# databio/gtars

Measured on AMD Instinct MI355X. Metric: query intervals/sec tokenized vs 100k-region hg38 universe, higher is better.
Workload: dtype u32; 1 GPU; BASELINE config 2: tokenize hg38-shaped query regions vs 100k-region universe (Bits order, CSR u64 offsets + u32 token ids), inputs resident in HBM; universe_regions=100000, distinct_batches=32, resident_bytes_rotated=714602184

## Files before the change

### gtars_amd/csrc/tokenize_lds.hip

```cpp
#include "common.h"
#include "scan.h"

#include <mutex>

namespace gtars {

#ifndef GTARS_TOK_ABLATE
#define GTARS_TOK_ABLATE 0
#endif

__device__ __forceinline__ i64 overlap_bp_tok(u32 as, u32 ae, u32 bs, u32 be) {
    u32 mn = ae < be ? ae : be;
    u32 mx = as > bs ? as : bs;
    return (i64)mn - (i64)mx;
}

typedef u32 u32x4 __attribute__((ext_vector_type(4)));
typedef u32 u32x2 __attribute__((ext_vector_type(2)));
typedef u64 u64x2 __attribute__((ext_vector_type(2)));
__device__ __forceinline__ u32x4 ld_stream4(const u32 *p) { return __builtin_nontemporal_load(reinterpret_cast<const u32x4 *>(p)); }
__device__ __forceinline__ u32x2 ld_stream2(const u32 *p) { return __builtin_nontemporal_load(reinterpret_cast<const u32x2 *>(p)); }
__device__ __forceinline__ void st_stream2(u64 *p, u64 a, u64 b) {
    u64x2 v = {a, b};
    __builtin_nontemporal_store(v, reinterpret_cast<u64x2 *>(p));
}

#ifndef GTARS_TOK_FILL_U
#define GTARS_TOK_FILL_U 4
#endif
#ifndef GTARS_TOK_PRIO
#define GTARS_TOK_PRIO 0
#endif
#ifndef GTARS_TOK_LB_W1
#define GTARS_TOK_LB_W1 1
#endif
#ifndef GTARS_TOK_KEYS_U16
#define GTARS_TOK_KEYS_U16 1
#endif
#ifndef GTARS_TOK_SEARCH8
#define GTARS_TOK_SEARCH8 1
#endif
#ifndef GTARS_TOK_STAMPS
#define GTARS_TOK_STAMPS 0
#endif
#ifndef GTARS_TOK_UNIT2_EXACT
#define GTARS_TOK_UNIT2_EXACT 1
#endif
#if GTARS_TOK_STAMPS
__device__ unsigned long long g_tok_stamps[2][12];
#define TSTAMP(k)                                         \
    do {                                                  \
        const u64 _t = __builtin_amdgcn_s_memtime();      \
        ts_acc[k] += _t - ts_last;                        \
        ts_last = _t;                                     \
    } while (0)
#else
#define TSTAMP(k) \
    do {          \
    } while (0)
#endif

template <bool FILTER>
__device__ __forceinline__ bool hit_test(u32 s, u32 e, u32 qs, u32 qe, i32 min_bp) {
    bool hit = (s < qe) & (e > qs);
    if (FILTER) hit = hit && overlap_bp_tok(qs, qe, s, e) >= (i64)min_bp;
    return hit;
}

template <bool FILTER>
__device__ __forceinline__ u32 block_mask4(const uint4 &S, const uint4 &E, u32 qs, u32 qe, i32 min_bp) {
    u32 m = 0;
    m |= (hit_test<FILTER>(S.x, E.x, qs, qe, min_bp) ? 1u : 0u);
    m |= (hit_test<FILTER>(S.y, E.y, qs, qe, min_bp) ? 1u : 0u) << 1;
    m |= (hit_test<FILTER>(S.z, E.z, qs, qe, min_bp) ? 1u : 0u) << 2;
    m |= (hit_test<FILTER>(S.w, E.w, qs, qe, min_bp) ? 1u : 0u) << 3;
    return m;
}

constexpr u32 B0_BITS = 22;
constexpr u32 B0_MASK = (1u << B0_BITS) - 1u;
__device__ __forceinline__ u32 run_state(u32 n, u32 m) { return (n & B0_MASK) | (m << B0_BITS) | ((n >> B0_BITS) << (B0_BITS + 4)); }
#ifndef GTARS_TOK_STAGE_RUNS
#define GTARS_TOK_STAGE_RUNS 1
#endif
constexpr u32 RUN_Q_BIT = 4, STAB_W_BIT = 8, STAB_N_BIT = 16;
__device__ __forceinline__ u32 run_state_n(u32 st) { return (st & B0_MASK) | ((st >> (B0_BITS + 4)) << B0_BITS); }

template <bool FILTER, u32 STRIDE, class F>
__device__ __forceinline__ u32 walk_tail(const uint4 *__restrict__ recs, u32 b0, u32 be, u32 qs, u32 qe, i32 min_bp, F &&f) {
    static_assert(ACC_OWN == 2, "a record = two own intervals + two look-ahead intervals");
    u32 n = 0;
    bool mr = true;
    for (u32 b = b0 + 2; mr && b < be; b += 2) {
        const uint4 S = recs[(size_t)b * STRIDE], E = recs[(size_t)b * STRIDE + 1];
        u32 m = block_mask4<FILTER>(S, E, qs, qe, min_bp);
        mr = S.w < qe;
        n += __popc(m);
        while (m) {
            const int k = __ffs((int)m) - 1;
            m &= m - 1;
            f(b, k);
        }
    }
    return n;
}

template <int SUB, bool IN_UNIT = true>
__device__ __forceinline__ void search_blocks(const AccelView &a, const u32 *s_lut, const u32 *s_q, const uint4 *s_ctab,
// ... 541 lines not shown
                }
            }
        } else {
            i = __popc(m);
        }
        if (more && want_ids) {
            const u32 n_tail = walk_tail<FILTER, STRIDE>(recs, b_tail, be, sq, eq, min_bp, [&](u32 b, int k) {
                put(slot(i++), IMPL ? t.aux[IMPL ? j : 0] + (u32)ACC_OWN * (b - b0) + (u32)k : recw[b * 16u + 8u + (u32)k]);
            });
            if (!tail_counted) n_all += n_tail;
        }
        run += n_all;
    }
}

template <int QPT, bool REV>
__device__ __forceinline__ void coop_runs(const TileQ<QPT, true> &t, const u64 (&o4)[QPT], u64 wave_base, u32 *__restrict__ ovals,
                                          u64 cap, int lane) {
    static_assert(QPT == 4, "four runs per source lane");
    u32 S[QPT], N[QPT], K[QPT];
    u32 any_big = 0;
#pragma unroll
    for (int j = 0; j < QPT; ++j) {
        const u32 m = (t.st[j] >> B0_BITS) & 15u, pm = __popc(m), w = (t.more_bits >> (STAB_W_BIT + 2 * j)) & 3u,
                  n_stab = (t.more_bits >> (STAB_N_BIT + 4 * j)) & 15u;
        const bool joined = w == 0 && mask_joins_tail(m);
        const u32 n = run_state_n(t.st[j]) + (joined ? pm : 0u);
        const bool big = ((t.more_bits >> (RUN_Q_BIT + j)) & 1u) && n >= COOP_MIN;
        S[j] = (u32)(o4[j] - wave_base) + (REV || joined ? 0u : pm + n_stab);
        N[j] = big ? n : 0u;
        const u32 id0 = joined ? t.aux[j] + (u32)(__ffs((int)m) - 1) : t.aux[j] + 4u + 4u * w;
        K[j] = REV ? id0 + (n - 1u) + S[j] : id0 - S[j];
        any_big |= N[j];
    }
    unsigned long long todo = __ballot(any_big != 0);
    if (!todo || wave_base >= cap) return;
    u32 *__restrict__ out = ovals + wave_base;
    const u32 room = cap - wave_base > 0xFFFFFFFFull ? 0xFFFFFFFFu : (u32)(cap - wave_base);
    u32 w0 = 0, val = 0;
    bool has = false;
    bool open = false;
    while (todo) {
        const int src = __ffsll((long long)todo) - 1;
        todo &= todo - 1;
        u32 s_[QPT], n_[QPT], k_[QPT];
#pragma unroll
        for (int j = 0; j < QPT; ++j) {
            s_[j] = (u32)__builtin_amdgcn_readlane((int)S[j], src);
            n_[j] = (u32)__builtin_amdgcn_readlane((int)N[j], src);
            k_[j] = (u32)__builtin_amdgcn_readlane((int)K[j], src);
        }
        u32 lo = 0xFFFFFFFFu, hi = 0;
#pragma unroll
        for (int j = 0; j < QPT; ++j)
            if (n_[j]) {
                lo = lo < s_[j] ? lo : s_[j];
                hi = s_[j] + n_[j];
            }
        hi = hi < room ? hi : room;
        for (u32 w = lo & ~63u; w < hi; w += 64) {
            if (w != w0) {
                if (open && has) __builtin_nontemporal_store(val, &out[w0 + (u32)lane]);
                has = false;
                w0 = w;
            }
            open = true;
            const u32 x = w + (u32)lane;
#pragma unroll
            for (int j = 0; j < QPT; ++j) {
                const bool in = x - s_[j] < n_[j];
                val = in ? (REV ? k_[j] - x : k_[j] + x) : val;
                has = has || in;
            }
            has = has && x < room;
        }
    }
    if (open && has) __builtin_nontemporal_store(val, &out[w0 + (u32)lane]);
}

template <int QPT, bool FILTER, bool IMPL, bool REV, int RUNS, bool U64 = false>
__device__ __forceinline__ void write_queries(const AccelView &a, const SearchLds &L, const u32 *__restrict__ qc,
                                              const u32 *__restrict__ qs, const u32 *__restrict__ qe, u64 nq, i32 min_bp,
                                              const TileQ<QPT, IMPL> &t, u64 q0, u64 wave_base, u64 *__restrict__ offsets,
                                              u32 *__restrict__ ovals, u64 cap, bool off_vec_ok, u32 *stage, u32 stage_cap,
                                              int lane) {
    const bool staged = cap && t.wtotal <= stage_cap && wave_base + t.wtotal <= cap;
    u64 o4[QPT];
    emit_queries<QPT, FILTER, IMPL, REV, RUNS, U64>(a, L, qc, qs, qe, min_bp, t, q0, wave_base + t.excl, cap != 0, o4, !staged, [&](u64 pos, u32 id) {
        if (GTARS_TOK_ABLATE & 2) return;
        if (staged)
            stage[(u32)(pos - wave_base)] = id;
        else if (pos < cap)
            ovals[pos] = id;
    });
    if constexpr (IMPL && !FILTER && (RUNS & 4) != 0) {
        if (!staged && cap && a.runs_ok && !(GTARS_TOK_ABLATE & (2 | 128))) coop_runs<QPT, REV>(t, o4, wave_base, ovals, cap, lane);
    }
    if (staged && !(GTARS_TOK_ABLATE & 2)) {
        for (u32 i = (u32)lane; i < t.wtotal; i += 64) __builtin_nontemporal_store(stage[i], &ovals[wave_base + i]);
    }
    if (GTARS_TOK_ABLATE & 4) {
        if (o4[0] == 0xFFFFFFFFFFFFFFFFull) offsets[q0] = o4[QPT - 1];
    } else if (QPT >= 2 && off_vec_ok && q0 + QPT <= nq) {
#pragma unroll
        for (int h = 0; h < QPT / 2; ++h) st_stream2(offsets + q0 + 2 * h, o4[2 * h], o4[2 * h + 1]);
    } else {
#pragma unroll
        for (int j = 0; j < QPT; ++j)
            if (q0 + j < nq) offsets[q0 + j] = o4[j];
    }
}

template <int QPT, bool FILTER, bool IMPL, bool REV, int RUNS, bool U64 = false>
__device__ __forceinline__ bool stage_queries(const AccelView &a, const SearchLds &L, const u32 *__restrict__ qc,
                                              const u32 *__restrict__ qs, const u32 *__restrict__ qe, i32 min_bp,
                                              const TileQ<QPT, IMPL> &t, u64 q0, u64 cap, u32 *stage, u32 stage_cap,
                                              u32 (&orel)[QPT]) {
    if (cap && t.wtotal > stage_cap) return false;
#if !GTARS_TOK_STAGE_RUNS
    if (IMPL && !FILTER && (RUNS & 1) && __ballot((t.more_bits >> RUN_Q_BIT) & 15u)) return false;
#endif
    u64 o4[QPT];
    emit_queries<QPT, FILTER, IMPL, REV, (GTARS_TOK_STAGE_RUNS != 0 ? RUNS : 0), U64>(a, L, qc, qs, qe, min_bp, t, q0, (u64)t.excl, cap != 0, o4, false, [&](u64 pos, u32 id) {
        if (GTARS_TOK_ABLATE & 2) return;
        stage[(u32)pos] = id;
    });
#pragma unroll
    for (int j = 0; j < QPT; ++j) orel[j] = (u32)o4[j];
    return true;
}
template <int QPT>
__device__ __forceinline__ void flush_queries(u64 nq, u32 wtotal, const u32 (&orel)[QPT], u64 q0, u64 wave_base,
                                              u64 *__restrict__ offsets, u32 *__restrict__ ovals, u64 cap, bool off_vec_ok,
                                              const u32 *stage, int lane) {
    if (cap && !(GTARS_TOK_ABLATE & 2)) {
        const u32 n = wave_base >= cap ? 0u : (cap - wave_base < (u64)wtotal ? (u32)(cap - wave_base) : wtotal);
        for (u32 i = (u32)lane; i < n; i += 64) __builtin_nontemporal_store(stage[i], &ovals[wave_base + i]);
    }
    if (GTARS_TOK_ABLATE & 4) {
        if (orel[0] == 0xFFFFFFFFu) offsets[q0] = orel[QPT - 1];
    } else if (QPT >= 2 && off_vec_ok && q0 + QPT <= nq) {
#pragma unroll
        for (int h = 0; h < QPT / 2; ++h) st_stream2(offsets + q0 + 2 * h, wave_base + orel[2 * h], wave_base + orel[2 * h + 1]);
    } else {
#pragma unroll
        for (int j = 0; j < QPT; ++j)
            if (q0 + j < nq) offsets[q0 + j] = wave_base + orel[j];
    }
}

template <bool FILTER>
__device__ __forceinline__ u64 help_count_tile(const AccelView &a, const SearchLds &L, const u32 *qc, const u32 *qs,
                                               const u32 *qe, u64 q_begin, u64 q_end, i32 min_bp) {
    u64 n = 0;
    for (u64 q = q_begin + (threadIdx.x & 63); q < q_end; q += 64) {
        const u32 c = qc[q], s = qs[q], e = qe[q];
        u32 b0, be;
        search_blocks<1>(a, L.lut, L.q, L.ctab, &c, &s, &b0, &be);
        if (b0 < be) {
            const uint4 S = a.rec2[(size_t)b0 * 2], E = a.rec2[(size_t)b0 * 2 + 1];
            n += __popc(block_mask4<FILTER>(S, E, s, e, min_bp));
            if (S.w < e && b0 + 2 < be) n += walk_tail<FILTER, 2>(a.rec2, b0, be, s, e, min_bp, [](u32, int) {});
        }
    }
    return wave_reduce_sum_u64(n);
}

template <int W, class Help>
__device__ __forceinline__ u64 resolve_prefix_helping(u64 *state, u32 tile, u64 agg, int lane, u32 epoch, u32 spin_limit,
                                                      u64 base, Help &&help) {
    const u64 ep = (u64)epoch << EP_SHIFT;
    u64 part = 0;
    i64 pred = (i64)tile - 1;
    u32 spins = 0;
    bool done = pred < 0;
    auto load_window = [&](i64 first) -> u64 {
        const i64 idx = first - lane;
        u64 v = ST_INC;
        if (idx >= 0) {
            v = ld_state(&state[idx]);
            if ((u32)((v >> EP_SHIFT) & EP_MAX) != epoch) v = 0;
        }
        return v;
    };
    while (!done) {
#if GTARS_TOK_STAMPS
        if (lane == 0) atomicAdd(&g_tok_stamps[1][spins ? 9 : 8], 1ull);
#endif
        u64 v[W];
#pragma unroll
        for (int w = 0; w < W; ++w) v[w] = load_window(pred - 64 * w);
#pragma unroll
        for (int w = 0; w < W; ++w) {
            if (done) continue;
            for (;;) {
                const u64 status = v[w] & ST_MASK;
                const unsigned long long b_inc = __ballot(status == ST_INC);
                const unsigned long long b_inv = __ballot(status == 0);
                const int first_inc = b_inc ? __ffsll((long long)b_inc) - 1 : 64;
                const unsigned long long need = first_inc >= 63 ? ~0ull : ((1ull << (first_inc + 1)) - 1ull);
                if (!(b_inv & need)) {
                    part += lane <= first_inc ? (v[w] & VAL_MASK) : 0ull;
                    if (first_inc < 64) done = true;
                    break;
                }
                if (++spins > spin_limit) {
                    const i64 missing = pred - 64 * w - (__ffsll((long long)(b_inv & need)) - 1);
                    const u64 h = help((u32)missing) + (missing == 0 ? base : 0ull);
                    if (lane == 0) st_state(&state[missing], (missing == 0 ? ST_INC : ST_AGG) | ep | h);
                    spins = 0;
                } else {
                    __builtin_amdgcn_s_sleep(1);
                }
                v[w] = load_window(pred - 64 * w);
            }
        }
        pred -= 64 * W;
        if (pred < 0) done = true;
    }
    const u64 excl = wave_reduce_sum_u48(part) + (tile == 0 ? base : 0ull);
    if (lane == 0) st_state(&state[tile], ST_INC | ep | (excl + agg));
    return excl;
}

__device__ __forceinline__ void group_barrier(u32 *ctr, u32 &phase, u32 members, int lane) {
    asm volatile("s_waitcnt lgkmcnt(0)" ::: "memory");
    phase += members;
    if (lane == 0) __hip_atomic_fetch_add(ctr, 1u, __ATOMIC_RELAXED, __HIP_MEMORY_SCOPE_WORKGROUP);
    for (;;) {
        const u32 v = __builtin_amdgcn_readfirstlane(__hip_atomic_load(ctr, __ATOMIC_RELAXED, __HIP_MEMORY_SCOPE_WORKGROUP));
        if ((i32)(v - phase) >= 0) break;
        __builtin_amdgcn_s_sleep(1);
    }
    asm volatile("" ::: "memory");
}

template <int TPB, int QPT, int R, int G, bool FILTER, bool IMPL, bool REV, int RUNS, bool U64 = false>
__global__ void __launch_bounds__(TPB, TPB / 256)
k_tok_lds(AccelView a, const u32 *__restrict__ qc, const u32 *__restrict__ qs, const u32 *__restrict__ qe,
          u64 nq, i32 min_bp, u64 *__restrict__ offsets, u32 *__restrict__ ovals, u64 cap, ScanWs *ws,
          u32 epoch, u32 ticket_base, u32 stage_cap, u32 spin_limit, const u64 *__restrict__ d_base,
          u64 *__restrict__ d_total_out) {
    extern __shared__ __attribute__((aligned(16))) u32 smem[];
    constexpr int NW = TPB / 64, GW = NW / G;
    static_assert(GW * R <= 64, "one lane per wave part in the group's scan");
    __shared__ u32 s_tile[G];
    __shared__ u64 s_prefix[G];
    __shared__ u32 s_scan[G][GW * R];
    __shared__ u32 s_bar[G];
    constexpr u32 ROUND = GW * 64 * QPT;
    constexpr u32 TILE = ROUND * R;

    const u32 num_tiles = (u32)((nq + TILE - 1) / TILE);
    const int lane = threadIdx.x & 63;
    const int wave = __builtin_amdgcn_readfirstlane(threadIdx.x >> 6);
    const int grp = wave / GW, gwave = wave % GW;
    const u32 gtid = threadIdx.x - (u32)grp * GW * 64;
    const u32 first_tiles = gridDim.x * G;
    const bool vec_ok = ((((uintptr_t)qc) | ((uintptr_t)qs) | ((uintptr_t)qe)) & 15u) == 0;
    const bool off_vec_ok = (((uintptr_t)offsets) & 15u) == 0;
    const SearchLds L = search_lds_view(a, smem);
    u32 *stage = smem + tok_lds_bytes(a) / 4 + (size_t)wave * stage_cap;
    const u64 base = d_base ? *d_base : 0ull;

    u32 c[R][QPT], s[R][QPT], e[R][QPT];
    auto load_tile = [&](u32 t) {
#pragma unroll
        for (int r = 0; r < R; ++r)
            load_queries<QPT>(qc, qs, qe, nq, (u64)t * TILE + (u64)r * ROUND + (u64)gtid * QPT, vec_ok, c[r], s[r], e[r]);
    };
    u32 tile = blockIdx.x * G + (u32)grp;
    load_tile(tile);
    if (G > 1 && threadIdx.x < G) s_bar[threadIdx.x] = 0;
    if (!(GTARS_TOK_ABLATE & 32)) fill_search_lds<TPB>(a, smem);
    __syncthreads();

    u32 phase = 0;
    auto bar = [&]() {
        if constexpr (G == 1)
            lds_barrier();
        else
            group_barrier(&s_bar[grp], phase, (u32)GW, lane);
    };
    auto help = [&](u32 t) -> u64 {
        const u64 qb = (u64)t * TILE, qn = qb + TILE < nq ? qb + TILE : nq;
        return help_count_tile<FILTER>(a, L, qc, qs, qe, qb, qn, min_bp);
    };

    struct Prev {
        TileQ<QPT, IMPL> q[R];
        u32 wbase[R], total, tile;
    } cur, prev;
    bool have_prev = false, loaded = true;
    const bool draw = num_tiles > first_tiles;
#if GTARS_TOK_STAMPS
    u64 ts_acc[12] = {0, 0, 0, 0, 0, 0, 0, 0, 0, 0, 0, 0}, ts_last = __builtin_amdgcn_s_memtime();
#endif
    for (;;) {
        const bool has_cur = tile < num_tiles;
        u32 next_tile = num_tiles;
        if (has_cur) {
            u32 ticket = 0;
            if (draw && gtid == 0) ticket = atomicAdd(&ws->ticket, 1u);
            if (!loaded) load_tile(tile);
            loaded = false;
#if GTARS_TOK_STAMPS
            asm volatile("s_waitcnt vmcnt(0)" ::: "memory");
#endif
            TSTAMP(0);
            u32 tsum[R], inc[R];
#if GTARS_TOK_PRIO & 1
            __builtin_amdgcn_s_setprio(1);
#endif
            count_rounds<R, QPT, FILTER, IMPL, REV, RUNS, U64>(a, L, c, s, e, min_bp, cur.q, tsum);
#if GTARS_TOK_PRIO & 1
            __builtin_amdgcn_s_setprio(0);
#endif
            TSTAMP(1);
#pragma unroll
            for (int r = 0; r < R; ++r) {
                inc[r] = wave_inclusive_scan_u32(tsum[r], lane);
                if (lane == 63) s_scan[grp][r * GW + gwave] = inc[r];
            }
            if (draw && gtid == 0) s_tile[grp] = first_tiles + (ticket - ticket_base);
            bar();
            TSTAMP(2);
            if (draw) next_tile = s_tile[grp];
            const u32 v = lane < GW * R ? s_scan[grp][lane] : 0u;
            const u32 vinc = wave_inclusive_scan_u32(v, lane);
            cur.total = __builtin_amdgcn_readlane(vinc, 63);
#pragma unroll
            for (int r = 0; r < R; ++r) {
                cur.q[r].wtotal = __builtin_amdgcn_readlane(v, r * GW + gwave);
                cur.wbase[r] = __builtin_amdgcn_readlane(vinc, r * GW + gwave) - cur.q[r].wtotal;
                cur.q[r].excl = inc[r] - tsum[r];
            }
            cur.tile = tile;
            if (gtid == 0) publish_aggregate(ws->state, tile, (u64)cur.total + (tile == 0 ? base : 0ull), epoch);
        }
        u32 orel0[QPT];
        bool pre0 = false;
        const u64 prev_q0 = (u64)prev.tile * TILE + (u64)gtid * QPT;
        if (have_prev && gwave != 0)
            pre0 = stage_queries<QPT, FILTER, IMPL, REV, RUNS, U64>(a, L, qc, qs, qe, min_bp, prev.q[0], prev_q0, cap, stage, stage_cap, orel0);
        if (have_prev && gwave == 0) {
            const u64 excl = (GTARS_TOK_ABLATE & 1) ? (u64)prev.tile * 2400u
                                                    : (draw ? resolve_prefix_helping<1>(ws->state, prev.tile, (u64)prev.total, lane, epoch, spin_limit, base, help)
                                                            : resolve_prefix_helping<GTARS_TOK_LB_W1>(ws->state, prev.tile, (u64)prev.total, lane, epoch,
                                                                                                      spin_limit, base, help));
            if (lane == 0) {
                s_prefix[grp] = excl;
                if (prev.tile == num_tiles - 1) {
                    offsets[nq] = excl + (u64)prev.total;
                    ws->total = excl + (u64)prev.total;
                    if (d_total_out) *d_total_out = excl + (u64)prev.total;
                }
            }
        }
        TSTAMP(7);
        if (have_prev) {
            if (gwave == 0)
                pre0 = stage_queries<QPT, FILTER, IMPL, REV, RUNS, U64>(a, L, qc, qs, qe, min_bp, prev.q[0], prev_q0, cap, stage, stage_cap, orel0);
            TSTAMP(3);
            bar();
            TSTAMP(4);
#if GTARS_TOK_PRIO & 2
            __builtin_amdgcn_s_setprio(1);
#endif
#pragma unroll
            for (int r = 0; r < R; ++r) {
                const u64 q0 = (u64)prev.tile * TILE + (u64)r * ROUND + (u64)gtid * QPT;
                if (r == 0 && pre0)
                    flush_queries<QPT>(nq, prev.q[0].wtotal, orel0, q0, s_prefix[grp] + prev.wbase[0], offsets, ovals, cap, off_vec_ok,
                                       stage, lane);
                else
                    write_queries<QPT, FILTER, IMPL, REV, RUNS, U64>(a, L, qc, qs, qe, nq, min_bp, prev.q[r], q0, s_prefix[grp] + prev.wbase[r],
                                                          offsets, ovals, cap, off_vec_ok, stage, stage_cap, lane);
            }
        }
#if GTARS_TOK_PRIO & 2
        __builtin_amdgcn_s_setprio(0);
#endif
        TSTAMP(5);
        bar();
        TSTAMP(6);
        if (!has_cur) break;
        prev = cur;
        have_prev = true;
        tile = next_tile;
    }
#if GTARS_TOK_STAMPS
    if (lane == 0 && wave < 2) {
        for (int k = 0; k < 11; ++k) atomicAdd(&g_tok_stamps[wave][k], ts_acc[k]);
        atomicAdd(&g_tok_stamps[wave][11], 1ull);
    }
#endif
}

constexpr u32 SWP_RUNS = 2;
constexpr u32 SWP_MASK_IV = 32;

template <bool FILTER>
__device__ __forceinline__ void sweep_query_global(const AccelView &a, u32 c, u32 s, u32 e, i32 min_bp, u32 &b0, u32 &mask, u32 &n,
                                                   bool &more) {
    const u32 bb = c ? a.chrom_tab[c - 1].w : 0u, be = a.chrom_tab[c].w;
    u32 lo = bb, hi = be;
    while (lo < hi) {
        const u32 mid = lo + ((hi - lo) >> 1);
        if (a.blk_first[mid] <= s)
            lo = mid + 1;
        else
            hi = mid;
    }
    b0 = lo;
    mask = 0;
    n = 0;
    more = false;
    u32 idx = 0;
    for (u32 b = lo; b < be; ++b, idx += 2) {
        const uint4 S = a.rec2[(size_t)b * 2], E = a.rec2[(size_t)b * 2 + 1];
        if (!(S.x < e)) break;
        const bool h0 = hit_test<FILTER>(S.x, E.x, s, e, min_bp);
        const bool go = S.y < e;
        const bool h1 = go && hit_test<FILTER>(S.y, E.y, s, e, min_bp);
        if (idx < SWP_MASK_IV)
            mask |= ((h0 ? 1u : 0u) | (h1 ? 2u : 0u)) << idx;
        else
            more = more || h0 || h1;
        n += (h0 ? 1u : 0u) + (h1 ? 1u : 0u);
        if (!go) break;
    }
}
template <bool FILTER, class F>
__device__ __forceinline__ void sweep_walk_from(const AccelView &a, u32 from, u32 be, u32 s, u32 e, i32 min_bp, F &&f) {
    for (u32 b = from; b < be; ++b) {
        const uint4 S = a.rec2[(size_t)b * 2], E = a.rec2[(size_t)b * 2 + 1];
        if (!(S.x < e)) break;
        if (hit_test<FILTER>(S.x, E.x, s, e, min_bp)) f(b, 0u);
        if (!(S.y < e)) break;
        if (hit_test<FILTER>(S.y, E.y, s, e, min_bp)) f(b, 1u);
    }
}
template <bool FILTER>
__device__ __forceinline__ u64 help_count_tile_sweep(const AccelView &a, const u32 *qc, const u32 *qs, const u32 *qe, u64 q_begin,
                                                     u64 q_end, i32 min_bp) {
    u64 n = 0;
    for (u64 q = q_begin + (threadIdx.x & 63); q < q_end; q += 64) {
        const u32 c = qc[q];
        if (c >= a.n_chrom) continue;
        u32 b0, m, k;
        bool more;
        sweep_query_global<FILTER>(a, c, qs[q], qe[q], min_bp, b0, m, k, more);
        n += k;
    }
    return wave_reduce_sum_u64(n);
}
__device__ __forceinline__ u32 wave_max_u32(u32 x) {
    x = max(x, (u32)__builtin_amdgcn_update_dpp(0, (int)x, 0x111, 0xf, 0xf, false));
    x = max(x, (u32)__builtin_amdgcn_update_dpp(0, (int)x, 0x112, 0xf, 0xf, false));
    x = max(x, (u32)__builtin_amdgcn_update_dpp(0, (int)x, 0x114, 0xf, 0xf, false));
// ... 297 lines not shown
        u32 wbase[R], total, tile;
    } cur, prev;
    bool have_prev = false;
    u32 tile = blockIdx.x;
    u64 ts_acc[12] = {0, 0, 0, 0, 0, 0, 0, 0, 0, 0, 0, 0}, ts_last = 0;
#if GTARS_TOK_STAMPS
    ts_last = __builtin_amdgcn_s_memtime();
#endif
    for (;;) {
        const bool has_cur = tile < num_tiles;
        u32 next_tile = num_tiles;
        if (has_cur) {
            u32 ticket = 0;
            if (draw && threadIdx.x == 0) ticket = atomicAdd(&ws->ticket, 1u);
            u32 tsum[R], inc[R];
            u32 c[QPT], s[QPT], e[QPT];
            load_queries<QPT>(qc, qs, qe, nq, (u64)tile * TILE + (u64)threadIdx.x * QPT, vec_ok, c, s, e);
#pragma unroll
            for (int r = 0; r < R; ++r) {
                u32 c2[QPT], s2[QPT], e2[QPT];
                if (r + 1 < R) load_queries<QPT>(qc, qs, qe, nq, (u64)tile * TILE + (u64)(r + 1) * ROUND + (u64)threadIdx.x * QPT, vec_ok, c2, s2, e2);
                tsum[r] = sweep_count_round<FILTER, IMPL>(a, c, s, e, min_bp, reg, cap_w, max_runs, lane, cur.q[r], ts_acc, ts_last);
                if (r + 1 < R) {
#pragma unroll
                    for (int j = 0; j < QPT; ++j) {
                        c[j] = c2[j];
                        s[j] = s2[j];
                        e[j] = e2[j];
                    }
                }
                inc[r] = wave_inclusive_scan_u32(tsum[r], lane);
                if (lane == 63) s_scan[r * NW + wave] = inc[r];
            }
            if (draw && threadIdx.x == 0) s_tile = first_tiles + (ticket - ticket_base);
            lds_barrier();
            TSTAMP(5);
            if (draw) next_tile = s_tile;
            const u32 v = lane < NW * R ? s_scan[lane] : 0u;
            const u32 vinc = wave_inclusive_scan_u32(v, lane);
            cur.total = __builtin_amdgcn_readlane(vinc, 63);
#pragma unroll
            for (int r = 0; r < R; ++r) {
                cur.q[r].wtotal = __builtin_amdgcn_readlane(v, r * NW + wave);
                cur.wbase[r] = __builtin_amdgcn_readlane(vinc, r * NW + wave) - cur.q[r].wtotal;
                cur.q[r].excl = inc[r] - tsum[r];
            }
            cur.tile = tile;
            if (threadIdx.x == 0) publish_aggregate(ws->state, tile, (u64)cur.total + (tile == 0 ? base : 0ull), epoch);
        }
        u32 orel[QPT];
        auto stage_round = [&](int r) -> bool {
            if (cap && prev.q[r].wtotal > region_words) return false;
            u64 o4[QPT];
            emit_sweep<FILTER, IMPL, REV>(a, qc, qs, qe, min_bp, prev.q[r], (u64)prev.tile * TILE + (u64)r * ROUND + (u64)threadIdx.x * QPT,
                                          (u64)prev.q[r].excl, cap != 0, o4, [&](u64 pos, u32 id) { reg[(u32)pos] = id; });
#pragma unroll
            for (int j = 0; j < QPT; ++j) orel[j] = (u32)o4[j];
            return true;
        };
        bool pre0 = false;
        if (have_prev && wave != 0) pre0 = stage_round(0);
        if (have_prev && wave == 0) {
            const u64 excl = resolve_prefix_helping<1>(ws->state, prev.tile, (u64)prev.total, lane, epoch, spin_limit, base, help);
            if (lane == 0) {
                s_prefix = excl;
                if (prev.tile == num_tiles - 1) {
                    offsets[nq] = excl + (u64)prev.total;
                    ws->total = excl + (u64)prev.total;
                    if (d_total_out) *d_total_out = excl + (u64)prev.total;
                }
            }
            pre0 = stage_round(0);
        }
        TSTAMP(6);
        if (have_prev) {
            lds_barrier();
            TSTAMP(7);
#pragma unroll
            for (int r = 0; r < R; ++r) {
                const u64 q0 = (u64)prev.tile * TILE + (u64)r * ROUND + (u64)threadIdx.x * QPT;
                const u64 wave_base = s_prefix + prev.wbase[r];
                const bool staged = r == 0 ? pre0 : stage_round(r);
                if (staged) {
                    flush_queries<QPT>(nq, prev.q[r].wtotal, orel, q0, wave_base, offsets, ovals, cap, off_vec_ok, reg, lane);
                } else {
                    u64 o4[QPT];
                    emit_sweep<FILTER, IMPL, REV>(a, qc, qs, qe, min_bp, prev.q[r], q0, wave_base + prev.q[r].excl, cap != 0, o4,
                                                  [&](u64 pos, u32 id) {
                                                      if (pos < cap) ovals[pos] = id;
                                                  });
                    if (off_vec_ok && q0 + QPT <= nq) {
#pragma unroll
                        for (int h = 0; h < QPT / 2; ++h) st_stream2(offsets + q0 + 2 * h, o4[2 * h], o4[2 * h + 1]);
                    } else {
#pragma unroll
                        for (int j = 0; j < QPT; ++j)
                            if (q0 + j < nq) offsets[q0 + j] = o4[j];
                    }
                }
            }
        }
        TSTAMP(8);
        lds_barrier();
        TSTAMP(9);
        if (!has_cur) break;
        prev = cur;
        have_prev = true;
        tile = next_tile;
    }
#if GTARS_TOK_STAMPS
    if (lane == 0 && wave < 2) {
        for (int k = 0; k < 11; ++k) atomicAdd(&g_tok_stamps[wave][k], ts_acc[k]);
        atomicAdd(&g_tok_stamps[wave][11], 1ull);
    }
#endif
}

__device__ __forceinline__ void load_queries_bf4(const u32 *__restrict__ qc, const u32 *__restrict__ qs, const u32 *__restrict__ qe,
                                                 u64 nq, u64 q0, u32 (&c)[4], u32 (&s)[4], u32 (&e)[4]) {
    const u64 qa = q0 < nq ? q0 : 0;
    const u32x4 c4 = ld_stream4(qc + qa), s4 = ld_stream4(qs + qa), e4 = ld_stream4(qe + qa);
    c[0] = q0 + 0 < nq ? c4.x : GTARS_UNKNOWN_CHROM; c[1] = q0 + 1 < nq ? c4.y : GTARS_UNKNOWN_CHROM;
    c[2] = q0 + 2 < nq ? c4.z : GTARS_UNKNOWN_CHROM; c[3] = q0 + 3 < nq ? c4.w : GTARS_UNKNOWN_CHROM;
    s[0] = s4.x; s[1] = s4.y; s[2] = s4.z; s[3] = s4.w;
    e[0] = e4.x; e[1] = e4.y; e[2] = e4.z; e[3] = e4.w;
}


template <int TPB, bool FILTER, bool PF, bool MARK = false>
__global__ void __launch_bounds__(TPB, 4)
k_count_lds(AccelView a, const u32 *__restrict__ qc, const u32 *__restrict__ qs, const u32 *__restrict__ qe, u64 nq,
            i32 min_bp, u32 *__restrict__ counts, u8 *__restrict__ any, u32 *mark = nullptr) {
    extern __shared__ __attribute__((aligned(16))) u32 smem[];
    constexpr int QPT = 4;
    constexpr u64 TILE = (u64)TPB * QPT;
    const SearchLds L = search_lds_view(a, smem);
    const u64 num_tiles = (nq + TILE - 1) / TILE;
    u32 c[QPT], s[QPT], e[QPT];
    if constexpr (PF) load_queries_bf4(qc, qs, qe, nq, (u64)blockIdx.x * TILE + (u64)threadIdx.x * QPT, c, s, e);
    fill_search_lds<TPB>(a, smem);
    __syncthreads();
    for (u64 tile = blockIdx.x; tile < num_tiles; tile += gridDim.x) {
        const u64 q0 = tile * TILE + (u64)threadIdx.x * QPT;
        if constexpr (!PF) load_queries<QPT>(qc, qs, qe, nq, q0, false, c, s, e);
        u32 b0[QPT], be[QPT];
        uint4 S[QPT], E[QPT];
        bool act[QPT];
#pragma unroll
        for (int h0 = 0; h0 < QPT; h0 += 2) {
            search_blocks<2>(a, L.lut, L.q, L.ctab, c + h0, s + h0, b0 + h0, be + h0);
#pragma unroll
            for (int j = h0; j < h0 + 2; ++j) {
                act[j] = b0[j] < be[j];
                const uint4 *rec = a.rec2 + (size_t)(act[j] ? b0[j] : 0u) * 2;
                S[j] = rec[0];
                E[j] = rec[1];
            }
            __builtin_amdgcn_sched_barrier(0);
        }
        u32 c2[QPT], s2[QPT], e2[QPT];
        if constexpr (PF) {
            __builtin_amdgcn_sched_barrier(0);
            load_queries_bf4(qc, qs, qe, nq, (tile + gridDim.x) * TILE + (u64)threadIdx.x * QPT, c2, s2, e2);
            __builtin_amdgcn_sched_barrier(0);
        }
        u32 n[QPT];
        if constexpr (MARK) {
// ... 63 lines not shown
        if (dev < 0 || dev >= 64) return fail(GTARS_ERR_INTERNAL, "device ordinal out of range");
        std::lock_guard<std::mutex> g(mu);
        if (!done[dev]) {
            GT_HIP(hipFuncSetAttribute(fn, hipFuncAttributeMaxDynamicSharedMemorySize, (int)TOK_LDS_TOTAL));
            int c = 256;
            GT_HIP(hipDeviceGetAttribute(&c, hipDeviceAttributeMultiprocessorCount, dev));
            cus[dev] = c;
            done[dev] = true;
        }
        n_cus = cus[dev];
        return GTARS_OK;
    }
};

gtars_status launch_count_lds(const AccelView &a, const u32 *qc, const u32 *qs, const u32 *qe, u64 nq, int has_min,
                              i32 min_overlap, u32 *counts, u8 *any, hipStream_t st) {
    if (nq == 0) return GTARS_OK;
    constexpr int TPB = 1024;
    const size_t lds = tok_lds_bytes(a);
    const bool filter = has_min && min_overlap > 1;
    const i32 min_bp = has_min ? min_overlap : 0;
    const bool pf = ((((uintptr_t)qc) | ((uintptr_t)qs) | ((uintptr_t)qe)) & 15u) == 0;
    auto kern = filter ? (pf ? k_count_lds<TPB, true, true> : k_count_lds<TPB, true, false>)
                       : (pf ? k_count_lds<TPB, false, true> : k_count_lds<TPB, false, false>);
    static KernelSetup setup[4];
    int dev = 0, cus = 256;
    gtars_status s0 = setup[(filter ? 2 : 0) + (pf ? 1 : 0)].get(reinterpret_cast<const void *>(kern), dev, cus);
    if (s0) return s0;
    const u64 tiles = (nq + (u64)TPB * 4 - 1) / ((u64)TPB * 4);
    const unsigned grid = (unsigned)std::min<u64>(tiles, (u64)cus);
    ProfScope p("k_count_lds", st);
    hipLaunchKernelGGL(kern, dim3(grid), dim3(TPB), lds, st, a, qc, qs, qe, nq, min_bp, counts, any, (u32 *)nullptr);
    GT_HIP(hipGetLastError());
    return GTARS_OK;
}

gtars_status launch_mark_lds(const AccelView &a, const u32 *qc, const u32 *qs, const u32 *qe, u64 nq, int has_min, i32 min_overlap,
                             u32 *mark, hipStream_t st) {
    if (nq == 0) return GTARS_OK;
    constexpr int TPB = 1024;
    const size_t lds = tok_lds_bytes(a);
    const bool filter = has_min && min_overlap > 1;
    const i32 min_bp = has_min ? min_overlap : 0;
    auto kern = filter ? k_count_lds<TPB, true, false, true> : k_count_lds<TPB, false, false, true>;
    static KernelSetup setup[2];
    int dev = 0, cus = 256;
    gtars_status s0 = setup[filter ? 1 : 0].get(reinterpret_cast<const void *>(kern), dev, cus);
    if (s0) return s0;
    const u64 tiles = (nq + (u64)TPB * 4 - 1) / ((u64)TPB * 4);
    const unsigned grid = (unsigned)std::min<u64>(tiles, (u64)cus);
    ProfScope p("k_mark_lds", st);
    hipLaunchKernelGGL(kern, dim3(grid), dim3(TPB), lds, st, a, qc, qs, qe, nq, min_bp, (u32 *)nullptr, (u8 *)nullptr, mark);
    GT_HIP(hipGetLastError());
    return GTARS_OK;
}

static u64 tok_tile_queries(int tpb, int qpt) { return (u64)tpb * (u64)qpt; }

static int choose_rounds(u64 nq, int cus) {
    const int forced = env_int("GTARS_TOK_ROUNDS", 0);
    if (forced == 1 || forced == 2) return forced;
    return nq >= (u64)cus * 8192ull ? 2 : 1;
}
static int choose_groups(u64 nq, int cus) {
    const int forced = env_int("GTARS_TOK_GROUPS", 0);
    if (forced == 1 || forced == 2) return forced;
    return nq >= (u64)cus * 8192ull * 4ull ? 2 : 1;
}

size_t tokenize_lds_ws_bytes(u64 nq) {
    return scan_ws_bytes_for_tiles((nq + 1023) / 1024);
}

static u32 stage_words(const AccelView &a, int tpb, int per_cu) {
    const int forced = env_int("GTARS_TOK_STAGE", -1);
    const size_t search = tok_lds_bytes(a);
    const size_t budget = TOK_LDS_TOTAL / (size_t)per_cu;
    if (search >= budget) return 0;
    size_t w = (budget - search) / 4 / (size_t)(tpb / 64);
    w = std::min<size_t>(w, forced >= 0 ? (size_t)forced : 512) / 64 * 64;
    return w >= 128 ? (u32)w : 0u;
}

template <int TPB, int QPT, int R, int G, bool FILTER, bool IMPL, bool REV, int RUNS, bool U64 = false>
static gtars_status launch_tok_t(const AccelView &a, const u32 *qc, const u32 *qs, const u32 *qe, u64 nq,
                                 i32 min_bp, const EnumOut &out, ScanWs *ws, ScanEpoch &ep, const u64 *d_base, u64 *d_total_out,
                                 hipStream_t st) {
    static KernelSetup setup;
    int dev = 0, cus = 256;
    gtars_status s0 = setup.get(reinterpret_cast<const void *>(k_tok_lds<TPB, QPT, R, G, FILTER, IMPL, REV, RUNS, U64>), dev, cus);
    if (s0) return s0;
    const u32 stage = stage_words(a, TPB, 1);
    const size_t lds = tok_lds_bytes(a) + (size_t)stage * 4 * (TPB / 64);
    const u32 spin_limit = (u32)env_int("GTARS_TOK_SPIN_LIMIT", 4096);
    const u64 tile_q = tok_tile_queries(TPB / G, QPT * R);
    const u64 tiles = (nq + tile_q - 1) / tile_q;
    const u64 grid = std::min<u64>((u64)cus, (tiles + G - 1) / G);
    const u64 cap = out.vals ? out.capacity : 0;
    hipLaunchKernelGGL((k_tok_lds<TPB, QPT, R, G, FILTER, IMPL, REV, RUNS, U64>), dim3((unsigned)grid), dim3(TPB), lds, st, a, qc, qs, qe, nq,
                       min_bp, out.offsets, out.vals, cap, ws, ep.epoch, ep.ticket_base, stage, spin_limit, d_base, d_total_out);
    GT_HIP(hipGetLastError());
    if (tiles > grid * G) ep.ticket_base += (u32)tiles;
    return GTARS_OK;
}

gtars_status launch_tokenize_lds(const AccelView &a, const u32 *qc, const u32 *qs, const u32 *qe, u64 nq,
                                 int has_min, i32 min_overlap, const EnumOut &out, void *scan_ws,
                                 size_t scan_ws_bytes, ScanEpoch &ep, hipStream_t st, const u64 *d_base, u64 *d_total_out, bool reverse) {
    if (out.starts || out.ends) return fail(GTARS_ERR_INTERNAL, "the LDS tokenizer writes vals only");
    if (nq == 0) {
        if (d_base) {
            GT_HIP(hipMemcpyAsync(out.offsets, d_base, sizeof(u64), hipMemcpyDeviceToDevice, st));
            GT_HIP(hipMemcpyAsync(&((ScanHead *)scan_ws)->total, d_base, sizeof(u64), hipMemcpyDeviceToDevice, st));
            if (d_total_out) GT_HIP(hipMemcpyAsync(d_total_out, d_base, sizeof(u64), hipMemcpyDeviceToDevice, st));
        } else {
            GT_HIP(hipMemsetAsync(out.offsets, 0, sizeof(u64), st));
            GT_HIP(hipMemsetAsync(&((ScanHead *)scan_ws)->total, 0, sizeof(u64), st));
            if (d_total_out) GT_HIP(hipMemsetAsync(d_total_out, 0, sizeof(u64), st));
        }
        return GTARS_OK;
    }
    constexpr int TPB = 1024;
    int cus = 256;
    {
        int dev = 0;
        GT_HIP(hipGetDevice(&dev));
        static int cached[64] = {};
        if (dev >= 0 && dev < 64) {
            if (!cached[dev]) {
                int c = 256;
                GT_HIP(hipDeviceGetAttribute(&c, hipDeviceAttributeMultiprocessorCount, dev));
                cached[dev] = c;
            }
            cus = cached[dev];
        }
    }
    const bool impl = a.ids_affine != 0;
    const bool filter = has_min && min_overlap > 1;
    const u64 cap_ids = out.vals ? out.capacity : 0;
    const bool by_rule = cap_ids == 0 || cap_ids / WIDE_IDS_PER_QUERY >= nq;
    const bool want_wide = out.hint == GTARS_TOK_WIDE || (out.hint != GTARS_TOK_NARROW && by_rule);
    const bool wide = GTARS_TOK_RUNS != 0 && !filter && a.runs_ok && !cfg_flag("GTARS_TOK_NARROW") &&
                      (want_wide || cfg_flag("GTARS_TOK_WIDE"));
    prof_note_fact(wide ? "tok_build_wide" : "tok_build_narrow");
    int rounds = impl && !wide ? choose_rounds(nq, cus) : 1;
    int groups = choose_groups(nq, cus);
    const bool unit_rec = a.rec8 && a.top_shift == 1 && impl && !filter && !reverse && !wide;
    if (unit_rec) rounds = 1;
    prof_note_fact(unit_rec ? "tok_unit_records" : "tok_block_records");
    const u64 dense = std::max<u64>(a.max_chrom_n, 1);
    if (dense * tok_tile_queries(TPB / groups, 4 * rounds) > 0xFFFFFFFFull) rounds = 1;
    if (dense * tok_tile_queries(TPB / groups, 4 * rounds) > 0xFFFFFFFFull) groups = 2;
    if (dense * tok_tile_queries(TPB / groups, 4 * rounds) > 0xFFFFFFFFull)
        return fail(GTARS_ERR_INVALID_ARG, "index too dense: a tile of queries could have more than 2^32 - 1 hits");
    const u64 tile_q = tok_tile_queries(TPB / groups, 4 * rounds);
    const u64 tiles = (nq + tile_q - 1) / tile_q;
    if (tiles > 0xFFFFFFF0ull) return fail(GTARS_ERR_INVALID_ARG, "query batch too large for one launch");
    const size_t need = scan_ws_bytes_for_tiles(tiles);
    if (scan_ws_bytes < need) return fail(GTARS_ERR_INTERNAL, "fused scan workspace too small");
    if (ep.epoch == 0 || ep.epoch >= EP_MAX || need > ep.cleared_bytes) {
        GT_HIP(hipMemsetAsync(scan_ws, 0, scan_ws_bytes, st));
        ep.cleared_bytes = scan_ws_bytes;
        ep.epoch = 0;
        ep.ticket_base = 0;
    }
    ep.epoch += 1;
    const i32 min_bp = has_min ? min_overlap : 0;
    ScanWs *ws = (ScanWs *)scan_ws;
    if (!impl && !a.rec4) return fail(GTARS_ERR_INTERNAL, "index has no id records");
    ProfScope p("k_tok_lds", st);
#define GT_TOK_CASE(N, GG, F, I, V, W)                                                                                      \
    if (rounds == N && groups == GG && filter == F && impl == I && reverse == V && wide == (W != 0))                        \
        return launch_tok_t<TPB, 4, N, GG, F, I, V, W>(a, qc, qs, qe, nq, min_bp, out, ws, ep, d_base, d_total_out, st);
#define GT_TOK_GEOM(N, GG, I)                                                                                               \
    GT_TOK_CASE(N, GG, false, I, false, 0)                                                                                  \
    GT_TOK_CASE(N, GG, true, I, false, 0)                                                                                   \
    GT_TOK_CASE(N, GG, false, I, true, 0)                                                                                   \
    GT_TOK_CASE(N, GG, true, I, true, 0)
#define GT_TOK_WIDE(GG, I)                                                                                                  \
    GT_TOK_CASE(1, GG, false, I, false, GTARS_TOK_RUNS)                                                                     \
    GT_TOK_CASE(1, GG, false, I, true, GTARS_TOK_RUNS)
    if (unit_rec && groups == 1) return launch_tok_t<TPB, 4, 1, 1, false, true, false, 0, true>(a, qc, qs, qe, nq, min_bp, out, ws, ep, d_base, d_total_out, st);
    if (unit_rec && groups == 2) return launch_tok_t<TPB, 4, 1, 2, false, true, false, 0, true>(a, qc, qs, qe, nq, min_bp, out, ws, ep, d_base, d_total_out, st);
    GT_TOK_GEOM(1, 1, true)
    GT_TOK_GEOM(2, 1, true)
    GT_TOK_GEOM(1, 2, true)
    GT_TOK_GEOM(2, 2, true)
    GT_TOK_GEOM(1, 1, false)
    GT_TOK_GEOM(1, 2, false)
#if GTARS_TOK_RUNS
    GT_TOK_WIDE(1, true)
    GT_TOK_WIDE(2, true)
    GT_TOK_WIDE(1, false)
    GT_TOK_WIDE(2, false)
#endif
#undef GT_TOK_WIDE
#undef GT_TOK_GEOM
#undef GT_TOK_CASE
    return fail(GTARS_ERR_INTERNAL, "unsupported tokenizer launch geometry");
}

bool tokenize_sweep_supported(const AccelView &a) {
    return a.n_blocks > 0 && a.rec2 && a.blk_first && a.chrom_tab && a.idc && (a.ids_affine || a.rec4) &&
           (u64)a.max_chrom_n * 4096ull <= 0xFFFFFFFFull;
}

template <int TPB, int R, bool FILTER, bool IMPL, bool REV>
static gtars_status launch_sweep_t(const AccelView &a, const u32 *qc, const u32 *qs, const u32 *qe, u64 nq, i32 min_bp, const EnumOut &out,
                                   ScanWs *ws, ScanEpoch &ep, const u64 *d_base, u64 *d_total_out, hipStream_t st) {
    static KernelSetup setup;
    int dev = 0, cus = 256;
    gtars_status s0 = setup.get(reinterpret_cast<const void *>(k_tok_sweep<TPB, R, FILTER, IMPL, REV>), dev, cus);
    if (s0) return s0;
    const u32 cap_w = (u32)std::min(486, std::max(1, env_int("GTARS_TOK_SWEEP_BLOCKS", 486)));
    const u32 max_runs = (u32)std::min<int>((int)SWP_RUNS, std::max(0, env_int("GTARS_TOK_SWEEP_RUNS", (int)SWP_RUNS)));
    const u32 region_words = 2432;
    const size_t lds = (size_t)region_words * (TPB / 64) * 4;
    const u32 spin_limit = (u32)env_int("GTARS_TOK_SPIN_LIMIT", 4096);
    const u64 tile_q = (u64)TPB * 4 * R;
    const u64 tiles = (nq + tile_q - 1) / tile_q;
    const u64 grid = std::min<u64>((u64)cus * (1024 / TPB), tiles);
    const u64 cap = out.vals ? out.capacity : 0;
    hipLaunchKernelGGL((k_tok_sweep<TPB, R, FILTER, IMPL, REV>), dim3((unsigned)grid), dim3(TPB), lds, st, a, qc, qs, qe, nq, min_bp,
                       out.offsets, out.vals, cap, ws, ep.epoch, ep.ticket_base, region_words, spin_limit, d_base, d_total_out, cap_w, max_runs);
    GT_HIP(hipGetLastError());
    if (tiles > grid) ep.ticket_base += (u32)tiles;
    return GTARS_OK;
}

gtars_status launch_tokenize_sweep(const AccelView &a, const u32 *qc, const u32 *qs, const u32 *qe, u64 nq, int has_min, i32 min_overlap,
                                   const EnumOut &out, void *scan_ws, size_t scan_ws_bytes, ScanEpoch &ep, hipStream_t st,
                                   const u64 *d_base, u64 *d_total_out, bool reverse) {
    if (out.starts || out.ends) return fail(GTARS_ERR_INTERNAL, "the sweep tokenizer writes vals only");
    if (nq == 0)
        return launch_tokenize_lds(a, qc, qs, qe, nq, has_min, min_overlap, out, scan_ws, scan_ws_bytes, ep, st, d_base, d_total_out, reverse);
    const bool impl = a.ids_affine != 0;
    const bool filter = has_min && min_overlap > 1;
    int cus = 256;
    {
        int dev = 0;
        GT_HIP(hipGetDevice(&dev));
        GT_HIP(hipDeviceGetAttribute(&cus, hipDeviceAttributeMultiprocessorCount, dev));
    }
    const int tpb = env_int("GTARS_TOK_SWEEP_TPB", 256) == 1024 && !filter && impl && !reverse ? 1024 : 256;
    int rounds = !filter && nq >= (u64)cus * 8192ull * 2ull ? 2 : 1;
    {
        const int forced = env_int("GTARS_TOK_SWEEP_ROUNDS", 0);
        if (forced == 1 || (forced == 2 && !filter)) rounds = forced;
    }
    if ((u64)std::max<u32>(a.max_chrom_n, 1) * 4ull * (u64)tpb * (u64)rounds > 0xFFFFFFFFull) rounds = 1;
    const u64 tile_q = 4ull * (u64)tpb * (u64)rounds;
    const u64 tiles = (nq + tile_q - 1) / tile_q;
    if (tiles > 0xFFFFFFF0ull) return fail(GTARS_ERR_INVALID_ARG, "query batch too large for one launch");
    const size_t need = scan_ws_bytes_for_tiles(tiles);
    if (scan_ws_bytes < need) return fail(GTARS_ERR_INTERNAL, "fused scan workspace too small");
    if (ep.epoch == 0 || ep.epoch >= EP_MAX || need > ep.cleared_bytes) {
        GT_HIP(hipMemsetAsync(scan_ws, 0, scan_ws_bytes, st));
        ep.cleared_bytes = scan_ws_bytes;
        ep.epoch = 0;
        ep.ticket_base = 0;
    }
    ep.epoch += 1;
    const i32 min_bp = has_min ? min_overlap : 0;
    ScanWs *ws = (ScanWs *)scan_ws;
    prof_note_fact("tok_build_sweep");
// ... 36 lines not shown
```

Baseline: 58.33 billion query intervals/s.

## Add one-tile-per-block tokenizer variant with early wave-0 staging and dense offset stores

Adds a ONE template specialization, used when rounds and groups are both 1 and the tile count fits within the CU count. In that case tiles are not drawn dynamically, and wave 0 stages its queries before the block barrier rather than after the scan, so the emit overlaps with waiting on the decoupled lookback. It also adds a dense offset store path that uses permlane32_swap and ds_bpermute so a full wave writes contiguous 16-byte vectors across lanes. The cost is extra template instantiations, extra register state held across the barrier, and cross-lane permutes.

```diff
diff --git a/gtars_amd/csrc/tokenize_lds.hip b/gtars_amd/csrc/tokenize_lds.hip
--- a/gtars_amd/csrc/tokenize_lds.hip
+++ b/gtars_amd/csrc/tokenize_lds.hip
@@ -24,6 +24,26 @@
     u64x2 v = {a, b};
     __builtin_nontemporal_store(v, reinterpret_cast<u64x2 *>(p));
 }
+
+#ifndef GTARS_TOK_EARLY0
+#define GTARS_TOK_EARLY0 1
+#endif
+#ifndef GTARS_TOK_DENSE_OFF
+#define GTARS_TOK_DENSE_OFF 1
+#endif
+__device__ __forceinline__ void store_offsets_dense(u64 *__restrict__ woff, u64 wave_base, const u32 (&o)[4], int lane) {
+    const auto a = __builtin_amdgcn_permlane32_swap(o[0], o[2], false, false);
+    const auto b = __builtin_amdgcn_permlane32_swap(o[1], o[3], false, false);
+    u32 x[2] = {a[0], a[1]}, y[2] = {b[0], b[1]};
+    const int src = (((lane >> 1) + 32 * (lane & 1)) << 2);
+#pragma unroll
+    for (int k = 0; k < 2; ++k) {
+        x[k] = (u32)__builtin_amdgcn_ds_bpermute(src, (int)x[k]);
+        y[k] = (u32)__builtin_amdgcn_ds_bpermute(src, (int)y[k]);
+        st_stream2(woff + 128 * k + 2 * lane, wave_base + x[k], wave_base + y[k]);
+    }
+}
+__device__ __forceinline__ bool wave_full(u64 q0, u64 nq, int lane) { return q0 - 4u * (u64)lane + 256u <= nq; }
 
 #ifndef GTARS_TOK_FILL_U
 #define GTARS_TOK_FILL_U 4
@@ -731,7 +751,7 @@
 __device__ __forceinline__ void write_queries(const AccelView &a, const SearchLds &L, const u32 *__restrict__ qc,
                                               const u32 *__restrict__ qs, const u32 *__restrict__ qe, u64 nq, i32 min_bp,
                                               const TileQ<QPT, IMPL> &t, u64 q0, u64 wave_base, u64 *__restrict__ offsets,
-                                              u32 *__restrict__ ovals, u64 cap, bool off_vec_ok, u32 *stage, u32 stage_cap,
+                                              u32 *__restrict__ ovals, u64 cap, bool off_vec_ok, bool dense_ok, u32 *stage, u32 stage_cap,
                                               int lane) {
     const bool staged = cap && t.wtotal <= stage_cap && wave_base + t.wtotal <= cap;
     u64 o4[QPT];
@@ -750,6 +770,9 @@
     }
     if (GTARS_TOK_ABLATE & 4) {
         if (o4[0] == 0xFFFFFFFFFFFFFFFFull) offsets[q0] = o4[QPT - 1];
+    } else if (GTARS_TOK_DENSE_OFF && QPT == 4 && dense_ok && wave_full(q0, nq, lane)) {
+        const u32 orel[4] = {(u32)(o4[0] - wave_base), (u32)(o4[1] - wave_base), (u32)(o4[2] - wave_base), (u32)(o4[3] - wave_base)};
+        store_offsets_dense(offsets + (q0 - 4u * (u64)lane), wave_base, orel, lane);
     } else if (QPT >= 2 && off_vec_ok && q0 + QPT <= nq) {
 #pragma unroll
         for (int h = 0; h < QPT / 2; ++h) st_stream2(offsets + q0 + 2 * h, o4[2 * h], o4[2 * h + 1]);
@@ -780,7 +803,7 @@
 }
 template <int QPT>
 __device__ __forceinline__ void flush_queries(u64 nq, u32 wtotal, const u32 (&orel)[QPT], u64 q0, u64 wave_base,
-                                              u64 *__restrict__ offsets, u32 *__restrict__ ovals, u64 cap, bool off_vec_ok,
+                                              u64 *__restrict__ offsets, u32 *__restrict__ ovals, u64 cap, bool off_vec_ok, bool dense_ok,
                                               const u32 *stage, int lane) {
     if (cap && !(GTARS_TOK_ABLATE & 2)) {
         const u32 n = wave_base >= cap ? 0u : (cap - wave_base < (u64)wtotal ? (u32)(cap - wave_base) : wtotal);
@@ -788,6 +811,8 @@
     }
     if (GTARS_TOK_ABLATE & 4) {
         if (orel[0] == 0xFFFFFFFFu) offsets[q0] = orel[QPT - 1];
+    } else if (GTARS_TOK_DENSE_OFF && QPT == 4 && dense_ok && wave_full(q0, nq, lane)) {
+        store_offsets_dense(offsets + (q0 - 4u * (u64)lane), wave_base, orel, lane);
     } else if (QPT >= 2 && off_vec_ok && q0 + QPT <= nq) {
 #pragma unroll
         for (int h = 0; h < QPT / 2; ++h) st_stream2(offsets + q0 + 2 * h, wave_base + orel[2 * h], wave_base + orel[2 * h + 1]);
@@ -884,7 +909,7 @@
     asm volatile("" ::: "memory");
 }
 
-template <int TPB, int QPT, int R, int G, bool FILTER, bool IMPL, bool REV, int RUNS, bool U64 = false>
+template <int TPB, int QPT, int R, int G, bool FILTER, bool IMPL, bool REV, int RUNS, bool U64 = false, bool ONE = false>
 __global__ void __launch_bounds__(TPB, TPB / 256)
 k_tok_lds(AccelView a, const u32 *__restrict__ qc, const u32 *__restrict__ qs, const u32 *__restrict__ qe,
           u64 nq, i32 min_bp, u64 *__restrict__ offsets, u32 *__restrict__ ovals, u64 cap, ScanWs *ws,
@@ -941,7 +966,13 @@
         u32 wbase[R], total, tile;
     } cur, prev;
     bool have_prev = false, loaded = true;
-    const bool draw = num_tiles > first_tiles;
+    static_assert(!ONE || (R == 1 && G == 1), "the one-tile build: one round, one group");
+    const bool draw = !ONE && num_tiles > first_tiles;
+    const bool dense_ok = ONE && GTARS_TOK_DENSE_OFF != 0 && off_vec_ok;
+    constexpr bool EARLY = ONE && GTARS_TOK_EARLY0 != 0;
+    u32 orel_e[QPT] = {};
+    bool pre_e = false;
+    const bool early0 = EARLY && gwave == 0;
 #if GTARS_TOK_STAMPS
     u64 ts_acc[12] = {0, 0, 0, 0, 0, 0, 0, 0, 0, 0, 0, 0}, ts_last = __builtin_amdgcn_s_memtime();
 #endif
@@ -972,6 +1003,17 @@
                 if (lane == 63) s_scan[grp][r * GW + gwave] = inc[r];
             }
             if (draw && gtid == 0) s_tile[grp] = first_tiles + (ticket - ticket_base);
+            if constexpr (EARLY) {
+#pragma unroll
+            for (int j = 0; j < QPT; ++j) orel_e[j] = 0;
+            if (early0) {
+                cur.q[0].excl = inc[0] - tsum[0];
+                cur.q[0].wtotal = __builtin_amdgcn_readlane(inc[0], 63);
+                const u64 cur_q0 = (u64)tile * TILE + (u64)gtid * QPT;
+                pre_e = stage_queries<QPT, FILTER, IMPL, REV, RUNS, U64>(a, L, qc, qs, qe, min_bp, cur.q[0], cur_q0, cap, stage, stage_cap, orel_e);
+            }
+            TSTAMP(10);
+            }
             bar();
             TSTAMP(2);
             if (draw) next_tile = s_tile[grp];
@@ -1008,8 +1050,14 @@
         }
         TSTAMP(7);
         if (have_prev) {
-            if (gwave == 0)
-                pre0 = stage_queries<QPT, FILTER, IMPL, REV, RUNS, U64>(a, L, qc, qs, qe, min_bp, prev.q[0], prev_q0, cap, stage, stage_cap, orel0);
+            if (gwave == 0) {
+                if (EARLY && early0) {
+                    pre0 = pre_e;
+#pragma unroll
+                    for (int j = 0; j < QPT; ++j) orel0[j] = orel_e[j];
+                } else
+                    pre0 = stage_queries<QPT, FILTER, IMPL, REV, RUNS, U64>(a, L, qc, qs, qe, min_bp, prev.q[0], prev_q0, cap, stage, stage_cap, orel0);
+            }
             TSTAMP(3);
             bar();
             TSTAMP(4);
@@ -1020,11 +1068,11 @@
             for (int r = 0; r < R; ++r) {
                 const u64 q0 = (u64)prev.tile * TILE + (u64)r * ROUND + (u64)gtid * QPT;
                 if (r == 0 && pre0)
-                    flush_queries<QPT>(nq, prev.q[0].wtotal, orel0, q0, s_prefix[grp] + prev.wbase[0], offsets, ovals, cap, off_vec_ok,
+                    flush_queries<QPT>(nq, prev.q[0].wtotal, orel0, q0, s_prefix[grp] + prev.wbase[0], offsets, ovals, cap, off_vec_ok, dense_ok,
                                        stage, lane);
                 else
                     write_queries<QPT, FILTER, IMPL, REV, RUNS, U64>(a, L, qc, qs, qe, nq, min_bp, prev.q[r], q0, s_prefix[grp] + prev.wbase[r],
-                                                          offsets, ovals, cap, off_vec_ok, stage, stage_cap, lane);
+                                                          offsets, ovals, cap, off_vec_ok, dense_ok, stage, stage_cap, lane);
             }
         }
 #if GTARS_TOK_PRIO & 2
@@ -1488,7 +1536,7 @@
                 const u64 wave_base = s_prefix + prev.wbase[r];
                 const bool staged = r == 0 ? pre0 : stage_round(r);
                 if (staged) {
-                    flush_queries<QPT>(nq, prev.q[r].wtotal, orel, q0, wave_base, offsets, ovals, cap, off_vec_ok, reg, lane);
+                    flush_queries<QPT>(nq, prev.q[r].wtotal, orel, q0, wave_base, offsets, ovals, cap, off_vec_ok, false, reg, lane);
                 } else {
                     u64 o4[QPT];
                     emit_sweep<FILTER, IMPL, REV>(a, qc, qs, qe, min_bp, prev.q[r], q0, wave_base + prev.q[r].excl, cap != 0, o4,
@@ -1718,13 +1766,13 @@
     return w >= 128 ? (u32)w : 0u;
 }
 
-template <int TPB, int QPT, int R, int G, bool FILTER, bool IMPL, bool REV, int RUNS, bool U64 = false>
+template <int TPB, int QPT, int R, int G, bool FILTER, bool IMPL, bool REV, int RUNS, bool U64 = false, bool ONE = false>
 static gtars_status launch_tok_t(const AccelView &a, const u32 *qc, const u32 *qs, const u32 *qe, u64 nq,
                                  i32 min_bp, const EnumOut &out, ScanWs *ws, ScanEpoch &ep, const u64 *d_base, u64 *d_total_out,
                                  hipStream_t st) {
     static KernelSetup setup;
     int dev = 0, cus = 256;
-    gtars_status s0 = setup.get(reinterpret_cast<const void *>(k_tok_lds<TPB, QPT, R, G, FILTER, IMPL, REV, RUNS, U64>), dev, cus);
+    gtars_status s0 = setup.get(reinterpret_cast<const void *>(k_tok_lds<TPB, QPT, R, G, FILTER, IMPL, REV, RUNS, U64, ONE>), dev, cus);
     if (s0) return s0;
     const u32 stage = stage_words(a, TPB, 1);
     const size_t lds = tok_lds_bytes(a) + (size_t)stage * 4 * (TPB / 64);
@@ -1732,12 +1780,24 @@
     const u64 tile_q = tok_tile_queries(TPB / G, QPT * R);
     const u64 tiles = (nq + tile_q - 1) / tile_q;
     const u64 grid = std::min<u64>((u64)cus, (tiles + G - 1) / G);
+    if constexpr (ONE) {
+        if (tiles > grid * G) return launch_tok_t<TPB, QPT, R, G, FILTER, IMPL, REV, RUNS, U64, false>(a, qc, qs, qe, nq, min_bp, out, ws, ep, d_base, d_total_out, st);
+    }
     const u64 cap = out.vals ? out.capacity : 0;
-    hipLaunchKernelGGL((k_tok_lds<TPB, QPT, R, G, FILTER, IMPL, REV, RUNS, U64>), dim3((unsigned)grid), dim3(TPB), lds, st, a, qc, qs, qe, nq,
+    hipLaunchKernelGGL((k_tok_lds<TPB, QPT, R, G, FILTER, IMPL, REV, RUNS, U64, ONE>), dim3((unsigned)grid), dim3(TPB), lds, st, a, qc, qs, qe, nq,
                        min_bp, out.offsets, out.vals, cap, ws, ep.epoch, ep.ticket_base, stage, spin_limit, d_base, d_total_out);
     GT_HIP(hipGetLastError());
     if (tiles > grid * G) ep.ticket_base += (u32)tiles;
     return GTARS_OK;
+}
+
+template <int TPB, int QPT, int R, int G, bool FILTER, bool IMPL, bool REV, int RUNS, bool U64 = false>
+static gtars_status launch_tok_pick(bool one, const AccelView &a, const u32 *qc, const u32 *qs, const u32 *qe, u64 nq, i32 min_bp,
+                                    const EnumOut &out, ScanWs *ws, ScanEpoch &ep, const u64 *d_base, u64 *d_total_out, hipStream_t st) {
+    if constexpr (R == 1 && G == 1) {
+        if (one) return launch_tok_t<TPB, QPT, R, G, FILTER, IMPL, REV, RUNS, U64, true>(a, qc, qs, qe, nq, min_bp, out, ws, ep, d_base, d_total_out, st);
+    }
+    return launch_tok_t<TPB, QPT, R, G, FILTER, IMPL, REV, RUNS, U64, false>(a, qc, qs, qe, nq, min_bp, out, ws, ep, d_base, d_total_out, st);
 }
 
 gtars_status launch_tokenize_lds(const AccelView &a, const u32 *qc, const u32 *qs, const u32 *qe, u64 nq,
@@ -1804,10 +1864,11 @@
     const i32 min_bp = has_min ? min_overlap : 0;
     ScanWs *ws = (ScanWs *)scan_ws;
     if (!impl && !a.rec4) return fail(GTARS_ERR_INTERNAL, "index has no id records");
+    const bool one = rounds == 1 && groups == 1 && tiles <= (u64)cus;
     ProfScope p("k_tok_lds", st);
 #define GT_TOK_CASE(N, GG, F, I, V, W)                                                                                      \
     if (rounds == N && groups == GG && filter == F && impl == I && reverse == V && wide == (W != 0))                        \
-        return launch_tok_t<TPB, 4, N, GG, F, I, V, W>(a, qc, qs, qe, nq, min_bp, out, ws, ep, d_base, d_total_out, st);
+        return launch_tok_pick<TPB, 4, N, GG, F, I, V, W>(one, a, qc, qs, qe, nq, min_bp, out, ws, ep, d_base, d_total_out, st);
 #define GT_TOK_GEOM(N, GG, I)                                                                                               \
     GT_TOK_CASE(N, GG, false, I, false, 0)                                                                                  \
     GT_TOK_CASE(N, GG, true, I, false, 0)                                                                                   \
@@ -1816,7 +1877,7 @@
 #define GT_TOK_WIDE(GG, I)                                                                                                  \
     GT_TOK_CASE(1, GG, false, I, false, GTARS_TOK_RUNS)                                                                     \
     GT_TOK_CASE(1, GG, false, I, true, GTARS_TOK_RUNS)
-    if (unit_rec && groups == 1) return launch_tok_t<TPB, 4, 1, 1, false, true, false, 0, true>(a, qc, qs, qe, nq, min_bp, out, ws, ep, d_base, d_total_out, st);
+    if (unit_rec && groups == 1) return launch_tok_pick<TPB, 4, 1, 1, false, true, false, 0, true>(one, a, qc, qs, qe, nq, min_bp, out, ws, ep, d_base, d_total_out, st);
     if (unit_rec && groups == 2) return launch_tok_t<TPB, 4, 1, 2, false, true, false, 0, true>(a, qc, qs, qe, nq, min_bp, out, ws, ep, d_base, d_total_out, st);
     GT_TOK_GEOM(1, 1, true)
     GT_TOK_GEOM(2, 1, true)
```

Result: faster. 59.28 billion query intervals/s, median of 6 (+1.6%).
